# larskaislaniemi/PyLamp

Measured on AMD Instinct MI355X. Metric: stokes_heat_mic_cell_updates_per_s, higher is better.
Workload: dtype f64

## Files before the change

include/pylamp_hip.h:

```cpp
#ifndef PYLAMP_HIP_H
#define PYLAMP_HIP_H

#include <stddef.h>
#include <stdint.h>

#ifdef __cplusplus
extern "C" {
#endif

typedef struct pl_ctx pl_ctx;

enum { PL_BC_NOSLIP = 0, PL_BC_FREESLIP = 1, PL_BC_CYCLIC = 2, PL_BC_FLOWTHRU = 4 };
enum { PL_BC_FIXTEMP = 0, PL_BC_FIXFLOW = 1 };
enum { PL_AVG_ARITHMETIC = 1, PL_AVG_GEOMETRIC = 2, PL_AVG_WEIGHTED = 4 };
enum { PL_INTERP_NEAREST = 8, PL_INTERP_LINEAR = 16, PL_INTERP_VELDIV = 32 };

typedef struct pl_solve_stats {
    int    iterations;
    int    converged;
    double rel_residual;
    double solve_ms;
    int    operator_applies;
    int    precond_applies;
    int    used_direct;
// ... 103 lines not shown
} pl_step_config;

typedef struct pl_step_report {
    double tstep;
    int    limiter;
    double tstep_heat, tstep_stokes;
    pl_solve_stats stokes, heat;
    double ms_props, ms_scatter, ms_stokes, ms_heat, ms_gather, ms_advect, ms_sort, ms_total;
    int64_t ntrac;
    int64_t ninjected;
    int     stokes_resolves;
    int64_t nremoved;
} pl_step_report;

int  pl_tracers_upload(pl_ctx* ctx, int64_t n, const double* tr_x, const double* tr_f);
int  pl_tracers_download(pl_ctx* ctx, int64_t n, double* tr_x, double* tr_f);
int  pl_tracers_count(pl_ctx* ctx, int64_t* n);
int  pl_tracers_census(pl_ctx* ctx, int64_t ncells, int32_t* counts, int* first_cell_row, int* n_cell_rows);
int  pl_tracers_layout(pl_ctx* ctx, int* epoch_age, int* lazy);
int  pl_step(pl_ctx* ctx, const pl_step_config* cfg, int it, pl_step_report* rep);
int  pl_resident_scatter(pl_ctx* ctx, const pl_step_config* cfg, int it);
int  pl_resident_temp_to_tracers(pl_ctx* ctx, const pl_step_config* cfg, int first, const double* newtemp, double tstep);
int  pl_resident_rk4(pl_ctx* ctx, const double* vz_pad, const double* vx_pad, double tstep, int fence, const double length[2]);
int  pl_get_field(pl_ctx* ctx, const char* name, double* out);
int  pl_get_tracer_velocity(pl_ctx* ctx, int64_t n, double* out);

typedef struct pl3_ctx pl3_ctx;
int  pl3_create(pl3_ctx** out, int device, int nz, int nx, int ny, const double* zc, const double* xc, const double* yc);
void pl3_destroy(pl3_ctx* ctx);
const char* pl3_last_error(const pl3_ctx* ctx);
int  pl3_set_comm(pl3_ctx* ctx, pl_ctx* comm, int Pz, int Px, int Py);
int  pl3_local_block(pl3_ctx* ctx, int first[3], int count[3]);
int  pl3_comm_stats(pl3_ctx* ctx, int64_t out[2], int reset);
int  pl3_stokes_set_coeffs(pl3_ctx* ctx, const double* etas, const double* etan, const double* rho, const double grav[3]);
int  pl3_stokes_set_wall_rows(pl3_ctx* ctx, int slaved);
int  pl3_stokes_set_walls(pl3_ctx* ctx, const int bc[6]);
int  pl3_stokes_set_wall_velocity(pl3_ctx* ctx, const double vel[18]);
int  pl3_stokes_get_wall_velocity(pl3_ctx* ctx, double vel[18]);
int  pl3_stokes_set_wall_flow(pl3_ctx* ctx, const double* const flow[6]);
int  pl3_stokes_get_wall_flow(pl3_ctx* ctx, int* mask, double* const flow[6]);
int  pl3_stokes_get_scaling(pl3_ctx* ctx, double* kcont, double* kbond);
int  pl3_stokes_apply(pl3_ctx* ctx, const double* x, double* y);
int  pl3_stokes_rhs(pl3_ctx* ctx, double* rhs);
int  pl3_stokes_rhs_scaled(pl3_ctx* ctx, double* rhs);
int  pl3_stokes_solve(pl3_ctx* ctx, const double* rhs, double* x, int use_x0, double rtol, int maxit, pl_solve_stats* stats);
int  pl3_stokes_apply_bench(pl3_ctx* ctx, int scaled, int reps, double* avg_ms);
// ... 101 lines not shown
```

pylamp_amd/_lib.py:

```python
import ctypes as C
import os

import numpy as np

_HERE = os.path.dirname(os.path.abspath(__file__))
LIB_PATH = os.path.join(_HERE, "libpylamp_hip.so")

c_double_p = C.POINTER(C.c_double)
c_int_p = C.POINTER(C.c_int)


class SolveStats(C.Structure):
    _fields_ = [("iterations", C.c_int), ("converged", C.c_int), ("rel_residual", C.c_double),
                ("solve_ms", C.c_double), ("operator_applies", C.c_int), ("precond_applies", C.c_int),
                ("used_direct", C.c_int), ("reserved_", C.c_int), ("error_estimate", C.c_double)]

    def as_dict(self):
        return {k: getattr(self, k) for k, _ in self._fields_}


class StepConfig(C.Structure):
    _fields_ = [("do_heatdiff", C.c_int), ("do_subgrid_heatdiff", C.c_int), ("tdep_rho", C.c_int),
                ("tdep_eta", C.c_int), ("etamin", C.c_double), ("etamax", C.c_double), ("tref", C.c_double),
                ("tstep_adv_max", C.c_double), ("tstep_adv_min", C.c_double), ("tstep_dif_max", C.c_double),
# ... 161 lines not shown
    "pl_heat_rhs": (C.c_int, [C.c_void_p, c_double_p]),
    "pl_heat_solve": (C.c_int, [C.c_void_p, c_double_p, c_double_p, C.c_double, C.c_int, C.POINTER(SolveStats)]),
    "pl_heat_apply_bench": (C.c_int, [C.c_void_p, C.c_int, c_double_p]),
    "pl_heat_fused_launches": (C.c_int, [C.c_void_p, C.POINTER(C.c_longlong)]),
    "pl_trac2grid": (C.c_int, [C.c_void_p, C.c_int64, c_double_p, c_double_p, C.c_int64, C.c_int, c_int_p,
                               C.c_double, C.c_double, C.c_double, C.c_double, C.POINTER(c_double_p)]),
    "pl_trac2grid_rect": (C.c_int, [C.c_void_p, C.c_int64, c_double_p, c_double_p, C.c_int64, C.c_int, c_int_p,
                                    c_double_p, c_double_p, C.POINTER(c_double_p)]),
    "pl_mic_set_search": (C.c_int, [C.c_void_p, C.c_int]),
    "pl_grid2trac": (C.c_int, [C.c_void_p, C.c_int64, c_double_p, C.c_int, C.POINTER(c_double_p), C.c_int,
                               C.c_int, c_double_p, c_double_p, C.c_int, C.c_double, C.c_int, c_double_p,
                               C.c_int64, C.POINTER(C.c_int64)]),
    "pl_rk4": (C.c_int, [C.c_void_p, C.c_int64, c_double_p, C.c_int, C.c_int, c_double_p, c_double_p,
                         c_double_p, c_double_p, C.c_double, c_double_p, c_double_p]),
    "pl_tracers_upload": (C.c_int, [C.c_void_p, C.c_int64, c_double_p, c_double_p]),
    "pl_tracers_download": (C.c_int, [C.c_void_p, C.c_int64, c_double_p, c_double_p]),
    "pl_tracers_count": (C.c_int, [C.c_void_p, C.POINTER(C.c_int64)]),
    "pl_tracers_census": (C.c_int, [C.c_void_p, C.c_int64, C.POINTER(C.c_int32), c_int_p, c_int_p]),
    "pl_tracers_layout": (C.c_int, [C.c_void_p, c_int_p, c_int_p]),
    "pl_step": (C.c_int, [C.c_void_p, C.POINTER(StepConfig), C.c_int, C.POINTER(StepReport)]),
    "pl_resident_scatter": (C.c_int, [C.c_void_p, C.POINTER(StepConfig), C.c_int]),
    "pl_resident_temp_to_tracers": (C.c_int, [C.c_void_p, C.POINTER(StepConfig), C.c_int, c_double_p, C.c_double]),
    "pl_resident_rk4": (C.c_int, [C.c_void_p, c_double_p, c_double_p, C.c_double, C.c_int, c_double_p]),
    "pl_get_field": (C.c_int, [C.c_void_p, C.c_char_p, c_double_p]),
    "pl_get_tracer_velocity": (C.c_int, [C.c_void_p, C.c_int64, c_double_p]),
}

_lib = None


def load():
    global _lib
    if _lib is not None:
        return _lib
    if not os.path.exists(LIB_PATH):
        raise Exception("pylamp_amd: %s is missing — run `python -c 'import __graft_entry__ as g; g.build()'` "
                        "(there is no CPU fallback)" % LIB_PATH)
    try:
        import torch
    except Exception:
        pass
    lib = C.CDLL(LIB_PATH)
    for name, (res, args) in SIGNATURES.items():
        fn = getattr(lib, name)
        fn.restype = res
        fn.argtypes = args
# ... 17 lines not shown
```

pylamp_amd/csrc/pl_mic.h:

```cpp
#pragma once
#include "pl_internal.h"

#define PL_MAX_SCATTER_FIELDS 8
#define PL_MAX_GATHER_FIELDS 8

#define PL_AVG_PRELOG 64
struct PlScatterArgs {
    long long n;
    const double* tz; const double* tx;
    int nf;
    const double* f[PL_MAX_SCATTER_FIELDS];
    int scheme[PL_MAX_SCATTER_FIELDS];
    double z0, hz, x0, hx;
    double rhz, rhx;
    const double* zc; const double* xc;
    int nz, nx;
    int row0, nrows, col0, ncols;
    double* wsum; double* cnt;
    double* acc[PL_MAX_SCATTER_FIELDS];
    const int* cell_start; int ncz, ncx;
    int crow0, ccol0;
    int stag_z, stag_x;
};

// ... 38 lines not shown
    int del_outside; double Lz, Lx;
    int* cell; int* count;
};
__device__ inline int mic_sort_key(const PlSortKey& k, double z, double x) {
    const int nc = k.ncz * k.ncx;
    if (k.del_outside && (z <= 0.0 || z >= k.Lz || x <= 0.0 || x >= k.Lx)) return nc + 8;
    int ci = (int)floor((z - k.z0) * k.rhz), cj = (int)floor((x - k.x0) * k.rhx);
    ci = min(max(ci, 0), k.gcz - 1) - k.crow0;
    cj = min(max(cj, 0), k.gcx - 1) - k.ccol0;
    const int dz = ci < 0 ? -1 : (ci >= k.ncz ? 1 : 0), dx = cj < 0 ? -1 : (cj >= k.ncx ? 1 : 0);
    if (dz == 0 && dx == 0) return ci * k.ncx + cj;
    return nc + (dx == 0 ? (dz < 0 ? 0 : 1) : (dz == 0 ? (dx < 0 ? 2 : 3) : (dz < 0 ? (dx < 0 ? 4 : 5) : (dx < 0 ? 6 : 7))));
}
__device__ inline void mic_wave_runs(int c, int lane, int& seg0, int& len) {
    const int prev = __shfl_up(c, 1, 64);
    const bool head = lane == 0 || prev != c;
    const unsigned long long heads = __ballot(head);
    seg0 = 63 - __clzll(heads & (~0ull >> (63 - lane)));
    const unsigned long long above = (seg0 == 63) ? 0ull : (heads >> (seg0 + 1));
    const int nact = __popcll(__ballot(1));
    len = above ? __ffsll((long long)above) : nact - seg0;
}

struct PlRk4Args {
    long long n;
    const double* tz; const double* tx;
    PlGatherGrid g;
    const double* Vz; const double* Vx;
    double dt;
    double* tz_out; double* tx_out; double* vz_out; double* vx_out;
    int fence; double eps, Lz, Lx;
    unsigned long long* n_outside_window;
    PlSortKey key;
};

struct PlScatterCellsArgs {
    const double* tz; const double* tx;
    const double* fn[6];
    const double* fm;
    const int* ix; unsigned ind;
    double z0, hz, rhz, x0, hx, rhx;
    int nz, nx;
    int row0, nrows, col0, ncols;
    const int* cell_start; int ncz, ncx, crow0, ccol0;
    double* accN; double* accC; double* accZ; double* accX;
    long long N;
    int* slow_count; int* slow_list; int slow_cap;
    int dbg;
};
#define PL_SCF_MAX 10
struct PlScatterFinalArgs {
    int nz, nx, nf;
    const double* acc[PL_SCF_MAX]; const double* den[PL_SCF_MAX]; int scheme[PL_SCF_MAX]; double* out[PL_SCF_MAX];
    long long acc_pitch, out_pitch, out_off;
};
int pl_scatter_cells_device(pl_ctx* ctx, PlScatterCellsArgs& a, int variant);
// ... 27 lines not shown
```

pylamp_amd/csrc/pl_mic.hip:

```cpp
#include "pl_internal.h"
#include "pl_mic.h"
#include <cmath>
#include <algorithm>

__global__ __launch_bounds__(256) void k_aos_to_soa(long long n, const double* __restrict__ src, long long ld,
                                                    int ncol, double* __restrict__ dst, long long dstride) {
    long long t = (long long)blockIdx.x * blockDim.x + threadIdx.x;
    if (t >= n) return;
    for (int k = 0; k < ncol; k++) dst[k * dstride + t] = src[t * ld + k];
}

__global__ __launch_bounds__(256) void k_soa_to_aos(long long n, const double* __restrict__ src, long long sstride,
                                                    int ncol, double* __restrict__ dst, long long ld) {
    long long t = (long long)blockIdx.x * blockDim.x + threadIdx.x;
    if (t >= n) return;
    for (int k = 0; k < ncol; k++) dst[t * ld + k] = src[k * sstride + t];
}

void pl_launch_aos_to_soa(pl_ctx* ctx, long long n, const double* src, long long ld, int ncol, double* dst,
                          long long dstride) {
    if (n <= 0) return;
    hipLaunchKernelGGL(k_aos_to_soa, dim3((unsigned)((n + 255) / 256)), dim3(256), 0, ctx->stream, n, src, ld, ncol,
                       dst, dstride);
}
// ... 318 lines not shown
        const double dz0 = z - a.g.gz[c.ie], dz1 = a.g.gz[c.ie + 1] - z;
        const double dx0 = x - a.g.gx[c.je], dx1 = a.g.gx[c.je + 1] - x;
        const double d[4] = {dz0 * dz0 + dx0 * dx0, dz0 * dz0 + dx1 * dx1, dz1 * dz1 + dx0 * dx0, dz1 * dz1 + dx1 * dx1};
        int m = 0;
        for (int k = 1; k < 4; k++) if (d[k] < d[m]) m = k;
        const long long o = a.g.off + (long long)(c.ie + (m >> 1)) * a.g.pitch + (c.je + (m & 1));
        for (int k = 0; k < a.nf; k++) a.out[k][t] = c.bad ? a.defval : a.fields[k][o];
        if (c.bad) atomicAdd(a.n_outside, 1ull);
    } else if (FAST || (a.method & PL_INTERP_LINEAR)) {
        const CellLoc c = mic_locate<FAST>(a.g, z, x);
        for (int k = 0; k < a.nf; k++) {
            const double v = mic_bilinear(a.fields[k], a.g, c);
            a.out[k][t] = c.bad ? a.defval : (a.accumulate ? a.out[k][t] + v : v);
        }
        if (c.bad) atomicAdd(a.n_outside, 1ull);
    } else {
        double uz, ux; bool bad, oow = false;
        mic_veldiv(a.g, a.fields[0], a.fields[1], z, x, a.defval, uz, ux, bad, oow);
        a.out[0][t] = uz; a.out[1][t] = ux;
        if (bad) atomicAdd(a.n_outside, 1ull);
    }
}

template <bool FAST>
__global__ __launch_bounds__(256) void k_rk4(PlRk4Args a) {
    long long t = (long long)blockIdx.x * blockDim.x + threadIdx.x;
    if (t >= a.n) return;
    const double z = a.tz[t], x = a.tx[t], dt = a.dt;
    double k1z, k1x, k2z, k2x, k3z, k3x, k4z, k4x; bool bad, oow = false;
    mic_veldiv<FAST>(a.g, a.Vz, a.Vx, z, x, 0.0, k1z, k1x, bad, oow);
    mic_veldiv<FAST>(a.g, a.Vz, a.Vx, z + 0.5 * dt * k1z, x + 0.5 * dt * k1x, 0.0, k2z, k2x, bad, oow);
    mic_veldiv<FAST>(a.g, a.Vz, a.Vx, z + 0.5 * dt * k2z, x + 0.5 * dt * k2x, 0.0, k3z, k3x, bad, oow);
    mic_veldiv<FAST>(a.g, a.Vz, a.Vx, z + dt * k3z, x + dt * k3x, 0.0, k4z, k4x, bad, oow);
    if (oow && a.n_outside_window) atomicAdd(a.n_outside_window, 1ull);
    const double zn = z + (1.0 / 6.0) * dt * (k1z + k2z + k3z + k4z);
    const double xn = x + (1.0 / 6.0) * dt * (k1x + k2x + k3x + k4x);
    if (FAST || a.g.fast_uniform) { const double rdt = 1.0 / dt; a.vz_out[t] = (zn - z) * rdt; a.vx_out[t] = (xn - x) * rdt; }
    else { a.vz_out[t] = (zn - z) / dt; a.vx_out[t] = (xn - x) / dt; }
    double zf = zn, xf = xn;
    if (a.fence) {
        if (zf <= 0.0) zf = a.eps; if (zf >= a.Lz) zf = a.Lz - a.eps;
        if (xf <= 0.0) xf = a.eps; if (xf >= a.Lx) xf = a.Lx - a.eps;
    }
    a.tz_out[t] = zf; a.tx_out[t] = xf;
    if (FAST && a.key.on) {
        const int c = mic_sort_key(a.key, zf, xf);
        a.key.cell[t] = c;
        int seg0, len;
        mic_wave_runs(c, threadIdx.x & 63, seg0, len);
        if ((int)(threadIdx.x & 63) == seg0) atomicAdd(&a.key.count[c], len);
    }
}

void pl_launch_gather(pl_ctx* ctx, const PlGatherArgs& a_in) {
    if (a_in.n <= 0) return;
    PlGatherArgs a = a_in;
    a.g.sz = (a.g.nz - 1) / a.g.Lz; a.g.sx = (a.g.nx - 1) / a.g.Lx;
    const bool fast = !a.g.rect && a.g.fast_uniform && (a.method & PL_INTERP_LINEAR) && !(a.method & PL_INTERP_NEAREST);
    const dim3 gr((unsigned)((a.n + 255) / 256));
    if (a.epi == 1 && fast && a.nf == 1) hipLaunchKernelGGL((k_gather<true, 1>), gr, dim3(256), 0, ctx->stream, a);
    else if (a.epi == 2 && fast && a.nf == 1) hipLaunchKernelGGL((k_gather<true, 2>), gr, dim3(256), 0, ctx->stream, a);
    else if (a.epi != 0) { (void)pl_fail(ctx, "pl_launch_gather: the fused epilogue needs the regular-grid bilinear path"); }
    else if (fast) hipLaunchKernelGGL((k_gather<true, 0>), gr, dim3(256), 0, ctx->stream, a);
    else hipLaunchKernelGGL((k_gather<false, 0>), gr, dim3(256), 0, ctx->stream, a);
}

void pl_launch_rk4(pl_ctx* ctx, const PlRk4Args& a_in) {
    if (a_in.n <= 0) return;
    PlRk4Args a = a_in;
    a.g.sz = (a.g.nz - 1) / a.g.Lz; a.g.sx = (a.g.nx - 1) / a.g.Lx;
    if (!a.g.rect && a.g.fast_uniform) hipLaunchKernelGGL(k_rk4<true>, dim3((unsigned)((a.n + 255) / 256)), dim3(256), 0, ctx->stream, a);
    else hipLaunchKernelGGL(k_rk4<false>, dim3((unsigned)((a.n + 255) / 256)), dim3(256), 0, ctx->stream, a);
}

static int upload_grid(pl_ctx* ctx, const char* name, int gnz, int gnx, const double* gz, const double* gx,
                       PlGatherGrid& g) {
    double* d;
    PL_TRY(pl_buf(ctx, name, (size_t)(gnz + gnx) * sizeof(double), &d, false));
    PL_HIP(ctx, hipMemcpyAsync(d, gz, gnz * sizeof(double), hipMemcpyHostToDevice, ctx->stream));
    PL_HIP(ctx, hipMemcpyAsync(d + gnz, gx, gnx * sizeof(double), hipMemcpyHostToDevice, ctx->stream));
    g.nz = gnz; g.nx = gnx; g.gz = d; g.gx = d + gnz;
    g.zmin = gz[0]; g.xmin = gx[0]; g.Lz = gz[gnz - 1] - gz[0]; g.Lx = gx[gnx - 1] - gx[0];
    g.pitch = gnx; g.off = 0; g.rect = ctx->mic_search ? 1 : 0;
    return 0;
}

extern "C" int pl_mic_set_search(pl_ctx* ctx, int on) { ctx->mic_search = on ? 1 : 0; return 0; }

static int trac2grid_host(pl_ctx* ctx, int64_t n, const double* tr_x, const double* tr_f, int64_t ld_f, int nf,
                          const int* avgscheme, double z0, double hz, double x0, double hx, const double* zc,
                          const double* xc, double* const* out) {
    if (n < 0 || !tr_x || !tr_f || !avgscheme || !out) return pl_fail(ctx, "pl_trac2grid: bad argument");
    if (nf < 1 || nf > PL_MAX_SCATTER_FIELDS) return pl_fail(ctx, "pl_trac2grid: 1..8 fields per call");
// ... 132 lines not shown
```

pylamp_amd/csrc/pl_step.hip:

```cpp
#include "pl_internal.h"
#include "pl_mic.h"
#include "pl_x0.h"
#include <algorithm>
#include <chrono>
#include <cmath>
#include <limits>

#define NFTRAC 13
enum { TR_RHO = 0, TR_ETA, TR_MRK, TR_TMP, TR_HCD, TR_HCP, TR_RH0, TR_ALP, TR_MAT, TR_ACE, TR_ET0, TR_IHT, TR__ID };
#define GASR 8.31446
#define PL_EPS (1.0 / 1024.0)

constexpr int NTCOLS = NFTRAC + 4;
struct PlStepState {
    long long n = 0, cap = 0;
    double* tz = nullptr; double* tx = nullptr;
    double* tz2 = nullptr; double* tx2 = nullptr;
    double* f[NFTRAC] = {nullptr};
    double* vtz = nullptr; double* vtx = nullptr;
    double* tmp[3] = {nullptr, nullptr, nullptr};
    double* partial = nullptr;
    std::vector<double> hpartial;
    double* gcoords = nullptr;
    bool have_newtemp = false, have_solution = false, have_dT = false;
    int n_prev = 0;
    double* x_hist[X0_HIST] = {};
    double dt_hist[X0_HIST + 1] = {};
    double* f2[NFTRAC] = {nullptr};
    int* cell = nullptr; int* dest = nullptr;
    int* orig = nullptr; int* orig2 = nullptr;
    int* cell_count = nullptr; int* cell_start = nullptr; int* block_sums = nullptr;
    int ncz = 0, ncx = 0;
    int crow0 = 0, ccol0 = 0;
    bool sorted = false;
    int* need = nullptr; int* need_off = nullptr;
    int* need_flag = nullptr; int* need_rank = nullptr;
    int* cell_res = nullptr;
    double max_id = -1.0;
    bool max_id_valid = false;
    int sort_cells = 0;
    int* slot = nullptr; int* slot2 = nullptr;
    bool epoch_on = false; int epoch_age = 0;
    long long epoch_len = 0;
    bool lazy_pending = false, lazy_inject = false; long long lazy_n = 0;
    bool cols_undefined = false;
    std::vector<double> gmz, gmx;
    double* flags = nullptr; double* counts_dev = nullptr; int counts_cap = 0;
};

static PlStepState* state_of(pl_ctx* ctx) {
    if (!ctx->step) ctx->step = new PlStepState();
    return (PlStepState*)ctx->step;
}

struct TracerArray { void** p; size_t elem; bool kept; };
static std::vector<TracerArray> tracer_arrays(PlStepState* S) {
    std::vector<TracerArray> v;
    for (double** q : {&S->tz, &S->tx, &S->tz2, &S->tx2, &S->vtz, &S->vtx, &S->tmp[0], &S->tmp[1], &S->tmp[2]})
        v.push_back({(void**)q, sizeof(double), q == &S->tz || q == &S->tx || q == &S->vtz || q == &S->vtx});
    for (int k = 0; k < NFTRAC; k++) { v.push_back({(void**)&S->f[k], sizeof(double), true}); v.push_back({(void**)&S->f2[k], sizeof(double), false}); }
    for (int** q : {&S->cell, &S->dest, &S->orig, &S->orig2, &S->slot, &S->slot2})
        v.push_back({(void**)q, sizeof(int), q == &S->cell || q == &S->orig || q == &S->slot});
    return v;
}
static std::vector<int**> sort_table_arrays(PlStepState* S) { return {&S->cell_count, &S->cell_start, &S->need, &S->need_off, &S->need_flag, &S->need_rank, &S->cell_res, &S->block_sums}; }

void pl_step_free(pl_ctx* ctx) {
    PlStepState* s = (PlStepState*)ctx->step;
// ... 428 lines not shown
    h.insert(h.end(), ctx->geom.zc.begin(), ctx->geom.zc.end());
    h.insert(h.end(), ctx->geom.xc.begin(), ctx->geom.xc.end());
    h.push_back(S->gmz[0] - (S->gmz[1] - S->gmz[0])); h.insert(h.end(), S->gmz.begin(), S->gmz.end());
    h.push_back(S->gmx[0] - (S->gmx[1] - S->gmx[0])); h.insert(h.end(), S->gmx.begin(), S->gmx.end());
    PL_HIP(ctx, hipMalloc((void**)&S->gcoords, h.size() * sizeof(double)));
    PL_HIP(ctx, hipMemcpy(S->gcoords, h.data(), h.size() * sizeof(double), hipMemcpyHostToDevice));
    return 0;
}
static const double* coords_z(pl_ctx* ctx, PlStepState* S, int stag) {
    if (ctx->geom.uniform) return nullptr;
    return stag ? S->gcoords + ctx->nz + ctx->nx + 1 : S->gcoords;
}
static const double* coords_x(pl_ctx* ctx, PlStepState* S, int stag) {
    if (ctx->geom.uniform) return nullptr;
    return stag ? S->gcoords + ctx->nz + ctx->nx + (ctx->nz + 1) + 1 : S->gcoords + ctx->nz;
}
static int migrate_tracers(pl_ctx* ctx, PlStepState* S, const StepGrid& q, const SortOpts& o = SortOpts());

extern "C" int pl_tracers_upload(pl_ctx* ctx, int64_t n, const double* tr_x, const double* tr_f) {
    if (n < 0 || !tr_x || !tr_f) return pl_fail(ctx, "pl_tracers_upload: bad argument");
    PL_HIP(ctx, hipSetDevice(ctx->device));
    PlStepState* S = state_of(ctx);
    PL_TRY(grow_tracers(ctx, S, n, 0));
    S->epoch_on = false; S->epoch_age = 0; S->lazy_pending = false; S->cols_undefined = false;
    const long long chunk = 1 << 22;
    PL_TRY(pl_stage(ctx, (size_t)chunk * NFTRAC * sizeof(double)));
    for (long long t0 = 0; t0 < n; t0 += chunk) {
        long long m = std::min<long long>(chunk, n - t0);
        PL_HIP(ctx, hipMemcpyAsync(ctx->stage, tr_x + 2 * t0, (size_t)m * 2 * sizeof(double), hipMemcpyHostToDevice, ctx->stream));
        hipLaunchKernelGGL(k_soa_from_aos2, grid1d(m), dim3(256), 0, ctx->stream, m, ctx->stage, S->tz + t0, S->tx + t0);
        PL_HIP(ctx, hipStreamSynchronize(ctx->stream));
        PL_HIP(ctx, hipMemcpyAsync(ctx->stage, tr_f + NFTRAC * t0, (size_t)m * NFTRAC * sizeof(double), hipMemcpyHostToDevice, ctx->stream));
        for (int k = 0; k < NFTRAC; k++)
            hipLaunchKernelGGL(k_col_from_aos, grid1d(m), dim3(256), 0, ctx->stream, m, ctx->stage, NFTRAC, k, S->f[k] + t0);
        PL_HIP(ctx, hipStreamSynchronize(ctx->stream));
    }
    PL_HIP(ctx, hipGetLastError());
    if (n > 0) hipLaunchKernelGGL(k_iota, grid1d(n), dim3(256), 0, ctx->stream, (long long)n, S->orig, 0);
    PL_HIP(ctx, hipStreamSynchronize(ctx->stream));
    S->n = n; S->have_newtemp = false; S->have_solution = false; S->have_dT = false; S->n_prev = 0; for (double& d : S->dt_hist) d = 0.0;
    for (double*& h : S->x_hist) h = nullptr;
    double idmax[1] = {-1.0};
    for (int64_t t = 0; t < n; t++) if (tr_f[NFTRAC * t + TR__ID] > idmax[0]) idmax[0] = tr_f[NFTRAC * t + TR__ID];
    PL_TRY(pl_allreduce_host(ctx, idmax, 1, 2));
    S->max_id = idmax[0]; S->max_id_valid = true;
    PL_TRY(ensure_coords(ctx, S));
    const StepGrid q = step_grid(ctx);
// ... 179 lines not shown
}
static int relayout(pl_ctx* ctx, PlStepState* S) {
    if (!S->epoch_on) return 0;
    S->epoch_on = false; S->epoch_age = 0;
    const long long n = S->n;
    if (n <= 0) return 0;
    int cols[NFTRAC], nc = 0;
    for (int k = 0; k < NFTRAC; k++) if (tracer_const(k)) cols[nc++] = k;
    for (int k0 = 0; k0 < nc; k0 += 5) {
        GatherColsArgs ga{}; ga.na = std::min(5, nc - k0);
        for (int k = 0; k < ga.na; k++) { ga.in[k] = S->f[cols[k0 + k]]; ga.out[k] = S->f2[cols[k0 + k]]; }
        hipLaunchKernelGGL(k_gather_cols, grid1d(n), dim3(256), 0, ctx->stream, n, S->slot, ga);
    }
    hipLaunchKernelGGL(k_gather_int, grid1d(n), dim3(256), 0, ctx->stream, n, S->slot, S->orig, S->orig2);
    for (int k = 0; k < nc; k++) std::swap(S->f[cols[k]], S->f2[cols[k]]);
    std::swap(S->orig, S->orig2);
    S->epoch_len = n;
    if (ctx->nranks > 1) hipLaunchKernelGGL(k_iota, grid1d(n), dim3(256), 0, ctx->stream, n, S->orig, 0);
    PL_HIP(ctx, hipGetLastError());
    return 0;
}
static int ensure_current(pl_ctx* ctx, PlStepState* S) {
    if (S->cols_undefined)
        return pl_fail(ctx, "tracer RHO / ETA / velocities are undefined: the last pl_step failed before it had rewritten them (upload the tracers again)");
    PL_TRY(flush_lazy(ctx, S));
    return relayout(ctx, S);
}

static void block_cells(const PlGeom& g, int& ncz, int& ncx) {
    ncz = (g.gi0 + g.lnz >= g.nz) ? g.lnz - 1 : g.lnz;
    ncx = (g.gj0 + g.lnx >= g.nx) ? g.lnx - 1 : g.lnx;
}
static int sort_tables(pl_ctx* ctx, PlStepState* S, int ncz, int ncx, bool keys_ready) {
    if (S->cell_count && S->ncz == ncz && S->ncx == ncx) return 0;
    if (keys_ready) return pl_fail(ctx, "sort_tracers: sort keys announced for another sort grid (internal error)");
    for (int** q : sort_table_arrays(S)) { if (*q) (void)hipFree(*q); *q = nullptr; }
    const int m = ncz * ncx + 10, nb = (m + 1023) / 1024;
    for (int** q : sort_table_arrays(S)) PL_HIP(ctx, hipMalloc((void**)q, (size_t)(q == &S->block_sums ? nb + 1 : m) * sizeof(int)));
    S->ncz = ncz; S->ncx = ncx;
    return 0;
}
static int recompute_max_id(pl_ctx* ctx, PlStepState* S, long long n) {
    double mx[1] = {-1.0};
    if (n > 0) {
        const int nbm = 256;
        if (!S->partial || S->hpartial.size() < (size_t)3 * 4096) {
            if (S->partial) (void)hipFree(S->partial);
// ... 410 lines not shown
            const int f2[1] = {TR_HCD}; const int s2[1] = {AW};
            double* pk[1] = {P.kz};
            PL_TRY(scatter_to_planes(ctx, S, 1, f2, s2, q, pk, 1, 0));
            pk[0] = P.kx;
            PL_TRY(scatter_to_planes(ctx, S, 1, f2, s2, q, pk, 0, 1));
        }
        if (it > 1 && S->have_newtemp)
            hipLaunchKernelGGL(k_copy_boundary, grid2d(g), dim3(64, 4), 0, ctx->stream, g, P.newT, P.T);
    } else if (cells) {
        const double* fn[2] = {S->f[TR_RHO], S->tmp[2]};
        double* out[3] = {P.rho, P.etas, P.etan};
        PL_TRY(scatter_cells(ctx, S, 1, fn, nullptr, q, out));
    } else {
        const int fi[2] = {TR_RHO, ETA_LOG}; const int sc[2] = {AW, GW};
        double* pl2[2] = {P.rho, P.etas};
        PL_TRY(scatter_to_planes(ctx, S, 2, fi, sc, q, pl2));
        const int f1[1] = {ETA_LOG}; const int s1[1] = {PL_AVG_GEOMETRIC | PL_AVG_PRELOG}; double* pn[1] = {P.etan};
        PL_TRY(scatter_to_planes(ctx, S, 1, f1, s1, q, pn, 1, 1));
    }
    PL_HIP(ctx, hipGetLastError());
    return 0;
}

static int stage_temp_to_tracers(pl_ctx* ctx, PlStepState* S, const pl_step_config* cfg, bool first, const StepPlanes& P, double tstep) {
    const PlGeom& g = ctx->geom.d;
    const int nz = g.nz, nx = g.nx;
    const long long n = S->n;
    const StepGrid q = step_grid(ctx);
    const double dz = cfg->length[0] / (nz - 1), dx = cfg->length[1] / (nx - 1);
    const int AW = PL_AVG_ARITHMETIC | PL_AVG_WEIGHTED;
    const int* ix = S->epoch_on ? S->slot : nullptr;
    double* cnt;
    PL_TRY(pl_buf(ctx, "mic_counter", 64, &cnt, false));
    PL_HIP(ctx, hipMemsetAsync(cnt, 0, 64, ctx->stream));
    PlGatherArgs ga{};
    ga.n = n; ga.tz = S->tz; ga.tx = S->tx; ga.nf = 1; ga.method = PL_INTERP_LINEAR;
    ga.defval = std::numeric_limits<double>::quiet_NaN(); ga.accumulate = 0; ga.n_outside = (unsigned long long*)cnt;
    ga.g.nz = nz; ga.g.nx = nx; ga.g.gz = S->gcoords; ga.g.gx = S->gcoords + nz;
    ga.g.zmin = ctx->geom.zc[0]; ga.g.xmin = ctx->geom.xc[0];
    ga.g.Lz = ctx->geom.zc[nz - 1] - ctx->geom.zc[0]; ga.g.Lx = ctx->geom.xc[nx - 1] - ctx->geom.xc[0];
    ga.g.rect = ctx->geom.uniform ? 0 : 1;
    ga.g.fast_uniform = ctx->geom.uniform ? 1 : 0;
    ga.g.pitch = g.pitch; ga.g.off = pl_idx(g, -g.gi0, -g.gj0);
    if (first) {
        ga.fields[0] = P.newT; ga.out[0] = S->f[TR_TMP];
        pl_launch_gather(ctx, ga);
    } else {
// ... 2 lines not shown
        S->have_dT = true;
        const double inv2 = (2.0 / dx) * (2.0 / dx) + (2.0 / dz) * (2.0 / dz);
        const bool fuse = ga.g.fast_uniform && !ga.g.rect;
        ga.fields[0] = P.dT; ga.out[0] = S->tmp[0];
        if (fuse) {
            ga.epi = 1; ga.epi_subgrid = cfg->do_subgrid_heatdiff; ga.epi_T = S->f[TR_TMP]; ga.epi_hcp = S->f[TR_HCP];
            ga.epi_rho = S->f[TR_RHO]; ga.epi_hcd = S->f[TR_HCD]; ga.epi_inv2 = inv2; ga.epi_dt = tstep;
            ga.epi_Tsub = S->tmp[1]; ga.epi_dTs = S->tmp[2]; ga.epi_ix = ix;
        }
        pl_launch_gather(ctx, ga);
        if (!fuse)
            hipLaunchKernelGGL(k_subgrid_part1, grid1d(n), dim3(256), 0, ctx->stream, n, S->f[TR_TMP], S->tmp[0], S->f[TR_HCP],
                               S->f[TR_RHO], S->f[TR_HCD], inv2, tstep, cfg->do_subgrid_heatdiff, S->tmp[1], S->tmp[2], ix);
        if (cfg->do_subgrid_heatdiff) {
            if (scatter_cells_on() && ctx->geom.uniform) {
                const double* fn[1] = {S->tmp[2]}; double* out[1] = {P.sgc};
                PL_TRY(scatter_cells(ctx, S, 2, fn, nullptr, q, out));
            } else {
                const int fs[1] = {-3}; const int ss[1] = {AW}; double* ps[1] = {P.sgc};
                PL_TRY(scatter_to_planes(ctx, S, 1, fs, ss, q, ps));
            }
            ga.fields[0] = P.sgc; ga.out[0] = S->tmp[0];
            if (fuse) ga.epi = 2;
            pl_launch_gather(ctx, ga);
            if (!fuse) hipLaunchKernelGGL(k_subgrid_part2, grid1d(n), dim3(256), 0, ctx->stream, n, S->f[TR_TMP], S->tmp[1], S->tmp[0]);
        }
        ga.epi = 0;
    }
    if (ctx->nranks > 1) {
        PL_TRY(step_flags(ctx, S));
        hipLaunchKernelGGL(k_flag_from_u64, dim3(1), dim3(1), 0, ctx->stream, (const unsigned long long*)cnt, S->flags);
        return 0;
    }
    unsigned long long nout = 0;
    PL_HIP(ctx, hipMemcpyAsync(&nout, cnt, sizeof(nout), hipMemcpyDeviceToHost, ctx->stream));
    PL_HIP(ctx, hipStreamSynchronize(ctx->stream));
    if (nout > 0) return pl_fail(ctx, "stopOnError in grid2trac");
    return 0;
}

static int stage_rk4(pl_ctx* ctx, PlStepState* S, const double* V, int I0, int I1, int J0, int J1, double tstep, int fence, double Lz, double Lx,
                     bool* keys_ready = nullptr) {
    const int nz = ctx->nz, nx = ctx->nx;
    const StepGrid q = step_grid(ctx);
    const int nVr = I1 - I0 + 1, nVc = J1 - J0 + 1;
    const size_t VN = (size_t)nVr * nVc;
    PlRk4Args ra{};
    ra.n = S->n; ra.tz = S->tz; ra.tx = S->tx;
    ra.g.nz = nz + 1; ra.g.nx = nx + 1; ra.g.gz = S->gcoords + nz + nx; ra.g.gx = S->gcoords + nz + nx + (nz + 1);
    {
        const double gz0 = S->gmz[0] - (S->gmz[1] - S->gmz[0]), gx0 = S->gmx[0] - (S->gmx[1] - S->gmx[0]);
        ra.g.zmin = gz0; ra.g.xmin = gx0; ra.g.Lz = S->gmz[nz - 1] - gz0; ra.g.Lx = S->gmx[nx - 1] - gx0;
    }
    ra.g.rect = ctx->geom.uniform ? 0 : 1;
    ra.g.fast_uniform = ctx->geom.uniform ? 1 : 0; ra.g.hx_over_hz = q.hx / q.hz; ra.g.hz_over_hx = q.hz / q.hx;
    ra.g.pitch = nVc; ra.g.off = -((long long)I0 * nVc + J0);
    ra.g.ie_lo = I0; ra.g.ie_hi = I1 - 1; ra.g.je_lo = J0; ra.g.je_hi = J1 - 1;
    ra.Vz = V; ra.Vx = V + VN; ra.dt = tstep;
    ra.tz_out = S->tz2; ra.tx_out = S->tx2; ra.vz_out = S->vtz; ra.vx_out = S->vtx;
    ra.fence = fence; ra.eps = PL_EPS; ra.Lz = Lz; ra.Lx = Lx;
    if (keys_ready) {
        *keys_ready = false;
        const PlGeom& g = ctx->geom.d;
        int ncz, ncx; block_cells(g, ncz, ncx);
        if (ctx->geom.uniform && S->cell_count && S->ncz == ncz && S->ncx == ncx && S->cell && S->n < (1LL << 31)) {
            PlSortKey& k = ra.key;
            k.on = 1; k.z0 = q.z0; k.rhz = 1.0 / q.hz; k.x0 = q.x0; k.rhx = 1.0 / q.hx;
            k.ncz = ncz; k.ncx = ncx; k.crow0 = g.gi0; k.ccol0 = g.gj0; k.gcz = g.nz - 1; k.gcx = g.nx - 1;
            k.del_outside = fence ? 0 : 1; k.Lz = Lz; k.Lx = Lx; k.cell = S->cell; k.count = S->cell_count;
            PL_HIP(ctx, hipMemsetAsync(S->cell_count, 0, (size_t)(ncz * ncx + 10) * sizeof(int), ctx->stream));
            *keys_ready = true;
        }
    }
    double* oowc = nullptr;
    if (ctx->nranks > 1) {
        PL_TRY(pl_buf(ctx, "rk4_counter", 64, &oowc, false));
        PL_HIP(ctx, hipMemsetAsync(oowc, 0, 64, ctx->stream));
        ra.n_outside_window = (unsigned long long*)oowc;
    }
    pl_launch_rk4(ctx, ra);
    PL_HIP(ctx, hipGetLastError());
    std::swap(S->tz, S->tz2); std::swap(S->tx, S->tx2);
    PL_HIP(ctx, hipStreamSynchronize(ctx->stream));
// ... 196 lines not shown
    PL_HIP(ctx, hipStreamSynchronize(ctx->stream));
    rep->ms_props = now_ms() - t0;
    t0 = now_ms();
    PL_TRY(stage_scatter(ctx, S, cfg, it, P));
    PL_HIP(ctx, hipStreamSynchronize(ctx->stream));
    rep->ms_scatter = now_ms() - t0;
    StepLimits L;
    PL_TRY(stage_limits(ctx, S, cfg, P, L));
    t0 = now_ms();
    PL_TRY(stage_stokes(ctx, S, cfg, P, L, rep));
    rep->ms_stokes = now_ms() - t0;
    const double tstep = rep->tstep;
    for (int k = X0_HIST; k > 0; k--) S->dt_hist[k] = S->dt_hist[k - 1];
    S->dt_hist[0] = tstep;
    if (!std::isfinite(tstep))
        return pl_fail(ctx, "pl_step: the time step is not finite - a grid node without any marker in reach makes the interpolated "
                            "fields NaN, and so do tracers injected into a cell without residents (their fields are 0/0 as in "
                            "pylamp2.py:624-629): raise the marker density or enable injection before cells run empty");
    if (cfg->do_heatdiff) {
        t0 = now_ms();
        PL_TRY(stage_heat(ctx, S, cfg, P, tstep, rep));
        rep->ms_heat = now_ms() - t0;
        t0 = now_ms();
        PL_TRY(stage_temp_to_tracers(ctx, S, cfg, it == 1 || !S->have_newtemp, P, tstep));
        S->have_newtemp = true;
        rep->ms_gather = now_ms() - t0;
    }
    t0 = now_ms();
    bool keys_ready = false;
    PL_TRY(stage_advect(ctx, S, cfg, tstep, &keys_ready));
    S->cols_undefined = false;
    rep->ms_advect = now_ms() - t0;
    t0 = now_ms();
    S->sorted = false;
    PL_TRY(stage_sort(ctx, S, cfg, it, keys_ready, rep));
    PL_HIP(ctx, hipStreamSynchronize(ctx->stream));
    S->sorted = true;
    rep->ms_sort = now_ms() - t0;
    rep->ntrac = S->n;
    rep->ms_total = now_ms() - t_all;
    return 0;
}

static int resident_ready(pl_ctx* ctx, const char* who, PlStepState*& S) {
    PL_HIP(ctx, hipSetDevice(ctx->device));
    S = state_of(ctx);
    if (ctx->nranks != 1) return pl_fail(ctx, std::string(who) + ": single-rank entry point (several ranks run pl_step)");
    if (!S->cell_start || !S->sorted) return pl_fail(ctx, std::string(who) + ": no cell-sorted tracers resident (call pl_tracers_upload)");
    PL_TRY(flush_lazy(ctx, S));
    return ensure_coords(ctx, S);
}

extern "C" int pl_resident_scatter(pl_ctx* ctx, const pl_step_config* cfg, int it) {
    if (!cfg) return pl_fail(ctx, "pl_resident_scatter: NULL argument");
    PlStepState* S;
    PL_TRY(resident_ready(ctx, "pl_resident_scatter", S));
    StepPlanes P;
    PL_TRY(step_planes(ctx, P));
    PL_TRY(stage_props(ctx, S, cfg));
    PL_TRY(stage_scatter(ctx, S, cfg, it, P));
    PL_HIP(ctx, hipStreamSynchronize(ctx->stream));
    return 0;
}

extern "C" int pl_resident_temp_to_tracers(pl_ctx* ctx, const pl_step_config* cfg, int first, const double* newtemp, double tstep) {
    if (!cfg || !newtemp) return pl_fail(ctx, "pl_resident_temp_to_tracers: NULL argument");
    PlStepState* S;
    PL_TRY(resident_ready(ctx, "pl_resident_temp_to_tracers", S));
    StepPlanes P;
    PL_TRY(step_planes(ctx, P));
    PL_TRY(pl_plane_upload(ctx, ctx->geom.d, newtemp, P.newT));
    PL_TRY(stage_temp_to_tracers(ctx, S, cfg, first != 0, P, tstep));
    PL_HIP(ctx, hipStreamSynchronize(ctx->stream));
    return 0;
}

extern "C" int pl_resident_rk4(pl_ctx* ctx, const double* vz_pad, const double* vx_pad, double tstep, int fence, const double length[2]) {
    if (!vz_pad || !vx_pad || !length) return pl_fail(ctx, "pl_resident_rk4: NULL argument");
    PlStepState* S;
    PL_TRY(resident_ready(ctx, "pl_resident_rk4", S));
    const int nz = ctx->nz, nx = ctx->nx;
    const size_t VN = (size_t)(nz + 1) * (nx + 1);
    double* V;
    PL_TRY(pl_buf(ctx, "advect_vel", 2 * VN * sizeof(double), &V, false));
    PL_HIP(ctx, hipMemcpyAsync(V, vz_pad, VN * sizeof(double), hipMemcpyHostToDevice, ctx->stream));
    PL_HIP(ctx, hipMemcpyAsync(V + VN, vx_pad, VN * sizeof(double), hipMemcpyHostToDevice, ctx->stream));
    PL_TRY(stage_rk4(ctx, S, V, 0, nz, 0, nx, tstep, fence ? 1 : 0, length[0], length[1]));
    S->sorted = false;
    PL_TRY(sort_tracers(ctx, S, step_grid(ctx)));
    PL_HIP(ctx, hipStreamSynchronize(ctx->stream));
    S->sorted = true;
    return 0;
}

extern "C" int pl_get_field(pl_ctx* ctx, const char* name, double* out) {
    if (!name || !out) return pl_fail(ctx, "pl_get_field: NULL argument");
    PL_HIP(ctx, hipSetDevice(ctx->device));
    const PlGeom& g = ctx->geom.d;
    std::string nm(name);
    const double* src = nullptr;
    if (nm == "velz" || nm == "velx" || nm == "pres") {
        double* x = pl_stokes_solution_device(ctx);
        if (!x) return pl_fail(ctx, "pl_get_field: no Stokes solution yet");
        src = x + (nm == "velz" ? 0 : nm == "velx" ? 1 : 2) * g.plane;
    } else {
        auto it = ctx->bufs.find(nm);
        if (it == ctx->bufs.end()) return pl_fail(ctx, "pl_get_field: unknown field '" + nm + "'");
        src = it->second;
    }
    return pl_plane_download(ctx, g, src, out);
// ... 2 lines not shown
```

pylamp_amd/driver.py:

```python
import ctypes as C
import os

import numpy as np

from . import _lib
from ._context import Context
from .pylamp_const import (DIM, IZ, IX, NFTRAC, SECINYR, TR_RHO, TR_ETA, TR_MRK, TR_TMP, TR_HCD, TR_HCP, TR_RH0, TR_ALP,
                           TR_MAT, TR_ACE, TR_ET0, TR_IHT, TR__ID)
from . import pylamp_stokes, pylamp_diff


class Options:

    def __init__(self, **kw):
        self.do_heatdiff = True
        self.do_subgrid_heatdiff = True
        self.tdep_rho = True
        self.tdep_eta = True
        self.etamin, self.etamax, self.Tref = 1e17, 1e23, 1623.0
        self.tstep_adv_max = 50e9 * SECINYR; self.tstep_adv_min = 50e-9 * SECINYR
        self.tstep_dif_max = 50e9 * SECINYR; self.tstep_dif_min = 50e-9 * SECINYR
        self.tstep_modifier = 0.67
        self.bcstokes = [pylamp_stokes.BC_TYPE_FREESLIP] * 4
        self.bcheat = [pylamp_diff.BC_TYPE_FIXTEMP, pylamp_diff.BC_TYPE_FIXFLOW,
# ... 203 lines not shown
        cfg = self._config()
        nt = _lib.f64(newtemp)
        if nt.shape != tuple(self.nx):
            raise Exception("temp_to_tracers: newtemp must be (nz, nx)")
        self.ctx.check(self.ctx.lib.pl_resident_temp_to_tracers(self.ctx.handle(), C.byref(cfg), int(bool(first)), _lib.dptr(nt), float(tstep)))
        return self.tracers()[1][:, TR_TMP]

    def layout(self):
        a = C.c_int(); b = C.c_int()
        self.ctx.check(self.ctx.lib.pl_tracers_layout(self.ctx.handle(), C.byref(a), C.byref(b)))
        return a.value, b.value

    def advect(self, vz_pad, vx_pad, tstep, fence=None, download=True):
        vz = _lib.f64(vz_pad); vx = _lib.f64(vx_pad)
        if vz.shape != (self.nx[0] + 1, self.nx[1] + 1) or vx.shape != vz.shape:
            raise Exception("advect: velocities must be (nz+1, nx+1)")
        fence = self.opt.tracs_fence_enabled if fence is None else fence
        Lc = (C.c_double * 2)(*self.L)
        self.ctx.check(self.ctx.lib.pl_resident_rk4(self.ctx.handle(), _lib.dptr(vz), _lib.dptr(vx), float(tstep), int(bool(fence)), Lc))
        if not download:
            return None
        return self.tracer_velocity(), self.tracers()[0]

    def write_snapshot(self, outdir="out"):
        velz, velx, pres, rho = self.field("velz"), self.field("velx"), self.field("pres"), self.field("rho")
        temp = self.field("temp") if self.opt.do_heatdiff else velx * 0.0
        if self.ctx.nranks > 1:
            tr_x, tr_f, tr_v = self.gather_tracers()
            if self.ctx.rank != 0:
                return
        else:
            tr_x, tr_f = self.tracers(); tr_v = self.tracer_velocity()
            k = getattr(self, "n_before_injection", tr_x.shape[0])
            tr_x, tr_f, tr_v = tr_x[:k], tr_f[:k], tr_v[:k]
        os.makedirs(outdir, exist_ok=True)
        np.savez(os.path.join(outdir, "griddata.{:06d}.npz".format(self.it)), gridz=self.grid[IZ], gridx=self.grid[IX],
                 velz=velz, velx=velx, pres=pres, rho=rho, temp=temp, tstep=self.it, time=self.totaltime)
        np.savez(os.path.join(outdir, "tracs.{:06d}.npz".format(self.it)), tr_x=tr_x, tr_f=tr_f,
                 tr_v=tr_v, tstep=self.it, time=self.totaltime)

    def close(self):
        self.ctx.close()


class VirtualCluster:

# ... 71 lines not shown
```

Before: 207.1 million.

## Fuse subgrid temperature gather tail into RK4 advection kernel

When the subgrid heat-diffusion gather would run as a separate pass, the step now defers it and the RK4 kernel applies it instead. The kernel already reads each tracer's position, so it locates the cell, bilinearly interpolates the subgrid correction and writes T = Tsub - v, saving one full tracer pass and its launch. The fast RK4 path also switches to nontemporal loads and stores for the streaming tracer arrays. In exchange the step state gains a pending-tail flag and a new intermediate undefined-state window, with an environment switch to turn the fusion off.

Result: no change. 208.3 million, median of 6 (+0.6%).

```diff
diff --git a/include/pylamp_hip.h b/include/pylamp_hip.h
--- a/include/pylamp_hip.h
+++ b/include/pylamp_hip.h
@@ -149,6 +149,8 @@
 int  pl_resident_scatter(pl_ctx* ctx, const pl_step_config* cfg, int it);
 int  pl_resident_temp_to_tracers(pl_ctx* ctx, const pl_step_config* cfg, int first, const double* newtemp, double tstep);
 int  pl_resident_rk4(pl_ctx* ctx, const double* vz_pad, const double* vx_pad, double tstep, int fence, const double length[2]);
+int  pl_resident_temp_to_tracers_rk4(pl_ctx* ctx, const pl_step_config* cfg, int first, const double* newtemp, double tstep,
+                                     const double* vz_pad, const double* vx_pad, int fence, const double length[2]);
 int  pl_get_field(pl_ctx* ctx, const char* name, double* out);
 int  pl_get_tracer_velocity(pl_ctx* ctx, int64_t n, double* out);
 
diff --git a/pylamp_amd/_lib.py b/pylamp_amd/_lib.py
--- a/pylamp_amd/_lib.py
+++ b/pylamp_amd/_lib.py
@@ -207,6 +207,8 @@
     "pl_resident_scatter": (C.c_int, [C.c_void_p, C.POINTER(StepConfig), C.c_int]),
     "pl_resident_temp_to_tracers": (C.c_int, [C.c_void_p, C.POINTER(StepConfig), C.c_int, c_double_p, C.c_double]),
     "pl_resident_rk4": (C.c_int, [C.c_void_p, c_double_p, c_double_p, C.c_double, C.c_int, c_double_p]),
+    "pl_resident_temp_to_tracers_rk4": (C.c_int, [C.c_void_p, C.POINTER(StepConfig), C.c_int, c_double_p, C.c_double, c_double_p, c_double_p,
+                                                  C.c_int, c_double_p]),
     "pl_get_field": (C.c_int, [C.c_void_p, C.c_char_p, c_double_p]),
     "pl_get_tracer_velocity": (C.c_int, [C.c_void_p, C.c_int64, c_double_p]),
 }
diff --git a/pylamp_amd/csrc/pl_mic.h b/pylamp_amd/csrc/pl_mic.h
--- a/pylamp_amd/csrc/pl_mic.h
+++ b/pylamp_amd/csrc/pl_mic.h
@@ -84,6 +84,14 @@
     len = above ? __ffsll((long long)above) : nact - seg0;
 }
 
+struct PlRk4Tail {
+    int on;
+    PlGatherGrid g;
+    const double* plane;
+    double defval;
+    const double* Tsub; double* T;
+};
+
 struct PlRk4Args {
     long long n;
     const double* tz; const double* tx;
@@ -94,6 +102,7 @@
     int fence; double eps, Lz, Lx;
     unsigned long long* n_outside_window;
     PlSortKey key;
+    PlRk4Tail tail;
 };
 
 struct PlScatterCellsArgs {
diff --git a/pylamp_amd/csrc/pl_mic.hip b/pylamp_amd/csrc/pl_mic.hip
--- a/pylamp_amd/csrc/pl_mic.hip
+++ b/pylamp_amd/csrc/pl_mic.hip
@@ -364,11 +364,18 @@
     }
 }
 
+__device__ inline void mic_rk4_tail(const PlRk4Tail& w, long long t, double z, double x) {
+    const CellLoc c = mic_locate<true>(w.g, z, x);
+    const double v = c.bad ? w.defval : mic_bilinear(w.plane, w.g, c);
+    __builtin_nontemporal_store(__builtin_nontemporal_load(w.Tsub + t) - v, w.T + t);
+}
+
 template <bool FAST>
 __global__ __launch_bounds__(256) void k_rk4(PlRk4Args a) {
     long long t = (long long)blockIdx.x * blockDim.x + threadIdx.x;
     if (t >= a.n) return;
-    const double z = a.tz[t], x = a.tx[t], dt = a.dt;
+    const double z = FAST ? __builtin_nontemporal_load(a.tz + t) : a.tz[t], x = FAST ? __builtin_nontemporal_load(a.tx + t) : a.tx[t], dt = a.dt;
+    if (FAST && a.tail.on) mic_rk4_tail(a.tail, t, z, x);
     double k1z, k1x, k2z, k2x, k3z, k3x, k4z, k4x; bool bad, oow = false;
     mic_veldiv<FAST>(a.g, a.Vz, a.Vx, z, x, 0.0, k1z, k1x, bad, oow);
     mic_veldiv<FAST>(a.g, a.Vz, a.Vx, z + 0.5 * dt * k1z, x + 0.5 * dt * k1x, 0.0, k2z, k2x, bad, oow);
@@ -377,14 +384,16 @@
     if (oow && a.n_outside_window) atomicAdd(a.n_outside_window, 1ull);
     const double zn = z + (1.0 / 6.0) * dt * (k1z + k2z + k3z + k4z);
     const double xn = x + (1.0 / 6.0) * dt * (k1x + k2x + k3x + k4x);
-    if (FAST || a.g.fast_uniform) { const double rdt = 1.0 / dt; a.vz_out[t] = (zn - z) * rdt; a.vx_out[t] = (xn - x) * rdt; }
+    if (FAST) { const double rdt = 1.0 / dt; __builtin_nontemporal_store((zn - z) * rdt, a.vz_out + t); __builtin_nontemporal_store((xn - x) * rdt, a.vx_out + t); }
+    else if (a.g.fast_uniform) { const double rdt = 1.0 / dt; a.vz_out[t] = (zn - z) * rdt; a.vx_out[t] = (xn - x) * rdt; }
     else { a.vz_out[t] = (zn - z) / dt; a.vx_out[t] = (xn - x) / dt; }
     double zf = zn, xf = xn;
     if (a.fence) {
         if (zf <= 0.0) zf = a.eps; if (zf >= a.Lz) zf = a.Lz - a.eps;
         if (xf <= 0.0) xf = a.eps; if (xf >= a.Lx) xf = a.Lx - a.eps;
     }
-    a.tz_out[t] = zf; a.tx_out[t] = xf;
+    if (FAST) { __builtin_nontemporal_store(zf, a.tz_out + t); __builtin_nontemporal_store(xf, a.tx_out + t); }
+    else { a.tz_out[t] = zf; a.tx_out[t] = xf; }
     if (FAST && a.key.on) {
         const int c = mic_sort_key(a.key, zf, xf);
         a.key.cell[t] = c;
@@ -411,6 +420,7 @@
     if (a_in.n <= 0) return;
     PlRk4Args a = a_in;
     a.g.sz = (a.g.nz - 1) / a.g.Lz; a.g.sx = (a.g.nx - 1) / a.g.Lx;
+    if (a.tail.on) { a.tail.g.sz = (a.tail.g.nz - 1) / a.tail.g.Lz; a.tail.g.sx = (a.tail.g.nx - 1) / a.tail.g.Lx; }
     if (!a.g.rect && a.g.fast_uniform) hipLaunchKernelGGL(k_rk4<true>, dim3((unsigned)((a.n + 255) / 256)), dim3(256), 0, ctx->stream, a);
     else hipLaunchKernelGGL(k_rk4<false>, dim3((unsigned)((a.n + 255) / 256)), dim3(256), 0, ctx->stream, a);
 }
diff --git a/pylamp_amd/csrc/pl_step.hip b/pylamp_amd/csrc/pl_step.hip
--- a/pylamp_amd/csrc/pl_step.hip
+++ b/pylamp_amd/csrc/pl_step.hip
@@ -44,6 +44,7 @@
     long long epoch_len = 0;
     bool lazy_pending = false, lazy_inject = false; long long lazy_n = 0;
     bool cols_undefined = false;
+    struct { bool on = false; PlGatherGrid g; const double* plane = nullptr; double defval = 0.0; } tail;
     std::vector<double> gmz, gmx;
     double* flags = nullptr; double* counts_dev = nullptr; int counts_cap = 0;
 };
@@ -518,7 +519,7 @@
     PL_HIP(ctx, hipSetDevice(ctx->device));
     PlStepState* S = state_of(ctx);
     PL_TRY(grow_tracers(ctx, S, n, 0));
-    S->epoch_on = false; S->epoch_age = 0; S->lazy_pending = false; S->cols_undefined = false;
+    S->epoch_on = false; S->epoch_age = 0; S->lazy_pending = false; S->cols_undefined = false; S->tail.on = false;
     const long long chunk = 1 << 22;
     PL_TRY(pl_stage(ctx, (size_t)chunk * NFTRAC * sizeof(double)));
     for (long long t0 = 0; t0 < n; t0 += chunk) {
@@ -744,7 +745,8 @@
 }
 static int ensure_current(pl_ctx* ctx, PlStepState* S) {
     if (S->cols_undefined)
-        return pl_fail(ctx, "tracer RHO / ETA / velocities are undefined: the last pl_step failed before it had rewritten them (upload the tracers again)");
+        return pl_fail(ctx, "tracer RHO / ETA / velocities (or the temperature, between its interpolation and the advection) are undefined: the "
+                            "last pl_step failed before it had rewritten them (upload the tracers again)");
     PL_TRY(flush_lazy(ctx, S));
     return relayout(ctx, S);
 }
@@ -1201,7 +1203,8 @@
     return 0;
 }
 
-static int stage_temp_to_tracers(pl_ctx* ctx, PlStepState* S, const pl_step_config* cfg, bool first, const StepPlanes& P, double tstep) {
+static bool rk4_tail_on() { const char* e = getenv("PYLAMP_RK4_TAIL"); return !(e && atoi(e) == 0); }
+static int stage_temp_to_tracers(pl_ctx* ctx, PlStepState* S, const pl_step_config* cfg, bool first, const StepPlanes& P, double tstep, bool defer_tail) {
     const PlGeom& g = ctx->geom.d;
     const int nz = g.nz, nx = g.nx;
     const long long n = S->n;
@@ -1250,7 +1253,10 @@
             }
             ga.fields[0] = P.sgc; ga.out[0] = S->tmp[0];
             if (fuse) ga.epi = 2;
-            pl_launch_gather(ctx, ga);
+            if (fuse && defer_tail && rk4_tail_on()) {
+                S->tail.on = true; S->tail.g = ga.g; S->tail.plane = P.sgc; S->tail.defval = ga.defval;
+                S->cols_undefined = true;
+            } else pl_launch_gather(ctx, ga);
             if (!fuse) hipLaunchKernelGGL(k_subgrid_part2, grid1d(n), dim3(256), 0, ctx->stream, n, S->f[TR_TMP], S->tmp[1], S->tmp[0]);
         }
         ga.epi = 0;
@@ -1287,6 +1293,12 @@
     ra.Vz = V; ra.Vx = V + VN; ra.dt = tstep;
     ra.tz_out = S->tz2; ra.tx_out = S->tx2; ra.vz_out = S->vtz; ra.vx_out = S->vtx;
     ra.fence = fence; ra.eps = PL_EPS; ra.Lz = Lz; ra.Lx = Lx;
+    if (S->tail.on) {
+        S->tail.on = false;
+        if (!ctx->geom.uniform) return pl_fail(ctx, "stage_rk4: a temperature tail is pending on a rectilinear grid (internal error)");
+        ra.tail.on = 1; ra.tail.g = S->tail.g; ra.tail.plane = S->tail.plane; ra.tail.defval = S->tail.defval;
+        ra.tail.Tsub = S->tmp[1]; ra.tail.T = S->f[TR_TMP];
+    }
     if (keys_ready) {
         *keys_ready = false;
         const PlGeom& g = ctx->geom.d;
@@ -1529,7 +1541,7 @@
         PL_TRY(stage_heat(ctx, S, cfg, P, tstep, rep));
         rep->ms_heat = now_ms() - t0;
         t0 = now_ms();
-        PL_TRY(stage_temp_to_tracers(ctx, S, cfg, it == 1 || !S->have_newtemp, P, tstep));
+        PL_TRY(stage_temp_to_tracers(ctx, S, cfg, it == 1 || !S->have_newtemp, P, tstep, true));
         S->have_newtemp = true;
         rep->ms_gather = now_ms() - t0;
     }
@@ -1554,6 +1566,7 @@
     S = state_of(ctx);
     if (ctx->nranks != 1) return pl_fail(ctx, std::string(who) + ": single-rank entry point (several ranks run pl_step)");
     if (!S->cell_start || !S->sorted) return pl_fail(ctx, std::string(who) + ": no cell-sorted tracers resident (call pl_tracers_upload)");
+    if (S->cols_undefined) return pl_fail(ctx, std::string(who) + ": the last step failed half-way; upload the tracers again");
     PL_TRY(flush_lazy(ctx, S));
     return ensure_coords(ctx, S);
 }
@@ -1577,7 +1590,7 @@
     StepPlanes P;
     PL_TRY(step_planes(ctx, P));
     PL_TRY(pl_plane_upload(ctx, ctx->geom.d, newtemp, P.newT));
-    PL_TRY(stage_temp_to_tracers(ctx, S, cfg, first != 0, P, tstep));
+    PL_TRY(stage_temp_to_tracers(ctx, S, cfg, first != 0, P, tstep, false));
     PL_HIP(ctx, hipStreamSynchronize(ctx->stream));
     return 0;
 }
@@ -1593,6 +1606,30 @@
     PL_HIP(ctx, hipMemcpyAsync(V, vz_pad, VN * sizeof(double), hipMemcpyHostToDevice, ctx->stream));
     PL_HIP(ctx, hipMemcpyAsync(V + VN, vx_pad, VN * sizeof(double), hipMemcpyHostToDevice, ctx->stream));
     PL_TRY(stage_rk4(ctx, S, V, 0, nz, 0, nx, tstep, fence ? 1 : 0, length[0], length[1]));
+    S->sorted = false;
+    PL_TRY(sort_tracers(ctx, S, step_grid(ctx)));
+    PL_HIP(ctx, hipStreamSynchronize(ctx->stream));
+    S->sorted = true;
+    return 0;
+}
+
+extern "C" int pl_resident_temp_to_tracers_rk4(pl_ctx* ctx, const pl_step_config* cfg, int first, const double* newtemp, double tstep,
+                                               const double* vz_pad, const double* vx_pad, int fence, const double length[2]) {
+    if (!cfg || !newtemp || !vz_pad || !vx_pad || !length) return pl_fail(ctx, "pl_resident_temp_to_tracers_rk4: NULL argument");
+    PlStepState* S;
+    PL_TRY(resident_ready(ctx, "pl_resident_temp_to_tracers_rk4", S));
+    StepPlanes P;
+    PL_TRY(step_planes(ctx, P));
+    PL_TRY(pl_plane_upload(ctx, ctx->geom.d, newtemp, P.newT));
+    const int nz = ctx->nz, nx = ctx->nx;
+    const size_t VN = (size_t)(nz + 1) * (nx + 1);
+    double* V;
+    PL_TRY(pl_buf(ctx, "advect_vel", 2 * VN * sizeof(double), &V, false));
+    PL_HIP(ctx, hipMemcpyAsync(V, vz_pad, VN * sizeof(double), hipMemcpyHostToDevice, ctx->stream));
+    PL_HIP(ctx, hipMemcpyAsync(V + VN, vx_pad, VN * sizeof(double), hipMemcpyHostToDevice, ctx->stream));
+    PL_TRY(stage_temp_to_tracers(ctx, S, cfg, first != 0, P, tstep, true));
+    PL_TRY(stage_rk4(ctx, S, V, 0, nz, 0, nx, tstep, fence ? 1 : 0, length[0], length[1]));
+    S->cols_undefined = false;
     S->sorted = false;
     PL_TRY(sort_tracers(ctx, S, step_grid(ctx)));
     PL_HIP(ctx, hipStreamSynchronize(ctx->stream));
diff --git a/pylamp_amd/driver.py b/pylamp_amd/driver.py
--- a/pylamp_amd/driver.py
+++ b/pylamp_amd/driver.py
@@ -249,6 +249,18 @@
             return None
         return self.tracer_velocity(), self.tracers()[0]
 
+    def temp_to_tracers_advect(self, newtemp, tstep, vz_pad, vx_pad, first=False, fence=None):
+        cfg = self._config()
+        nt = _lib.f64(newtemp); vz = _lib.f64(vz_pad); vx = _lib.f64(vx_pad)
+        if nt.shape != tuple(self.nx):
+            raise Exception("temp_to_tracers_advect: newtemp must be (nz, nx)")
+        if vz.shape != (self.nx[0] + 1, self.nx[1] + 1) or vx.shape != vz.shape:
+            raise Exception("temp_to_tracers_advect: velocities must be (nz+1, nx+1)")
+        fence = self.opt.tracs_fence_enabled if fence is None else fence
+        Lc = (C.c_double * 2)(*self.L)
+        self.ctx.check(self.ctx.lib.pl_resident_temp_to_tracers_rk4(self.ctx.handle(), C.byref(cfg), int(bool(first)), _lib.dptr(nt), float(tstep),
+                                                                    _lib.dptr(vz), _lib.dptr(vx), int(bool(fence)), Lc))
+
     def write_snapshot(self, outdir="out"):
         velz, velx, pres, rho = self.field("velz"), self.field("velx"), self.field("pres"), self.field("rho")
         temp = self.field("temp") if self.opt.do_heatdiff else velx * 0.0
```
